# ShinYwings/SingleHDR-tf2

Hardware: AMD Instinct MI355X
Metric: HDR images/sec (512x512) end-to-end inference, deq+lin+hal (higher is better)
Workload: dtype f32

## Files before the change

### include/shdr.h

```cpp
#ifndef SHDR_H_
#define SHDR_H_

#include <stdint.h>

#ifdef __cplusplus
extern "C" {
#endif

void shdr_config_reload(void);

#define SHDR_OK          0
#define SHDR_E_SHAPE    (-1)
#define SHDR_E_ALIGN    (-2)
#define SHDR_E_ARCH     (-3)
#define SHDR_E_LAUNCH   (-4)
#define SHDR_E_NULL     (-5)

#define SHDR_ACT_NONE   0
#define SHDR_ACT_RELU   1
#define SHDR_ACT_LRELU  2
#define SHDR_ACT_TANH   3

#define SHDR_ALGO_AUTO    0
#define SHDR_ALGO_MFMA    1
// ... 163 lines not shown
                               int F, int K, void* stream);
int shdr_increase_bwd_f32(const float* rf, const float* dout, float* drf, int B, int K, void* stream);
int shdr_apply_rf_bwd_f32(const float* x, const float* rf, const float* dy, float* drf, float* dx,
                          int B, int64_t n_per_batch, int K, void* stream);
int shdr_diff_loss_f32(const float* a, const float* b, float* out, int B, int64_t n_per_sample,
                       int mode, void* stream);
int shdr_diff_loss_bwd_f32(const float* a, const float* b, const float* g, float* da, int B,
                           int64_t n_per_sample, int mode, int accumulate, void* stream);
int shdr_tv_loss_f32(const float* y, float* out, int N, int H, int W, int C, void* stream);
int shdr_tv_loss_bwd_f32(const float* y, const float* g, float* dy, int N, int H, int W, int C,
                         int accumulate, void* stream);
int shdr_logc_bwd_f32(const float* dy, const float* x, float* dx, int64_t n, void* stream);
int shdr_alpha_mask_f32(const float* x, float* alpha, int64_t npix, float thr, void* stream);
int shdr_alpha_blend_bwd_f32(const float* dA, const float* alpha, float* dhal, int64_t npix, void* stream);
int shdr_vgg_preprocess_bwd_f32(const float* dy, float* dx, int64_t npix, int in_channels, void* stream);
int shdr_adam_f32(float* p, const float* g, float* m, float* v, int64_t n, float lr_t, float beta1,
                  float beta2, float eps, float grad_scale, void* stream);

int shdr_winograd_filter_f32(const float* w, float* u, int Cin, int Cout, void* stream);
int64_t shdr_winograd_tiles(int N, int H, int W);
int shdr_winograd_input_f32(const float* x, float* v, int N, int H, int W, int C, void* stream);
int shdr_winograd_output_f32(const float* m, float* y, const float* bias, const float* scale,
                             const float* shift, int N, int H, int W, int C, int act1, int act2,
                             void* stream);

int shdr_lin_frontend_bwd_f32(const float* img, const float* dF, float* dimg, int N, int H, int W,
                              int y_channels, void* stream);
int shdr_alpha_blend_full_bwd_f32(const float* b, const float* hal, const float* dA, float* dB,
                                  float* dhal, int64_t npix, float thr, void* stream);
int shdr_unpack3_f32(const float* y, float* o0, float* o1, float* o2, float* o3, int nout,
                     int channels, int64_t npix, void* stream);
int shdr_sample_dot_f32(const float* a, const float* b, float* out, int B, int64_t n_per_sample, void* stream);
int shdr_mean_norm_fwd_f32(const float* r, const float* sum, float* out, int B, int64_t n_per_sample,
                           float eps, float target, void* stream);
int shdr_mean_norm_bwd_f32(const float* g, const float* sum, const float* gdot, float* dr, int B,
                           int64_t n_per_sample, float eps, float target, void* stream);

int shdr_act_bwd_bias_f32(const float* dy, const float* y, float* dz, float* db, float* ws, int64_t npix, int C, int act, void* stream);

int shdr_winograd_filter_packed_f32(const float* w, float* up, int Cin, int Cout, void* stream);
int shdr_conv2d_winograd_fused_f32(const float* x, const float* u, const float* bias, const float* scale,
                                   const float* shift, float* y, int N, int H, int W, int Cin, int Cout,
                                   int act1, int act2, void* stream);

int shdr_conv2d_winograd_fused2_f32(const float* x, const float* x2, const float* u, const float* bias,
                                    const float* scale, const float* shift, float* y, float* y_pool, int N, int H, int W,
                                    int C1, int C2, int Cout, int act1, int act2, void* stream);

int shdr_conv2d_winograd_fused_up2_f32(const float* x, const float* u, const float* bias, const float* scale,
                                       const float* shift, float* y, int N, int H, int W, int Cin, int Cout,
                                       int act1, int act2, void* stream);

int shdr_conv2d_x3_ok_f32(const shdr_conv2d_desc* d);
int64_t shdr_conv2d_x3_filter_elems_f32(const shdr_conv2d_desc* d);
int shdr_conv2d_x3_prepare_filter_f32(const shdr_conv2d_desc* d, const float* w, float* prepared, void* stream);
int shdr_conv2d_x3_input_absmax_f32(const float* x, int64_t n, float* prepared, void* stream);
int shdr_conv2d_fwd_x3_f32(const shdr_conv2d_desc* d, const float* x1, const float* x2, const float* prepared, const float* bias,
                           const float* scale, const float* shift, float* y, float* y_pool, void* stream);
int shdr_conv2d_fwd_x3_ranged_f32(const shdr_conv2d_desc* d, const float* x1, const float* x2, const float* prepared, const float* bias,
                                  const float* scale, const float* shift, float* y, float* y_pool, const float* x1_range,
                                  const float* x2_range, float* y_range, void* stream);
int shdr_conv2d_fwd_x3_residual_f32(const shdr_conv2d_desc* d, const float* x1, const float* x2, const float* prepared, const float* bias,
                                    const float* scale, const float* shift, const float* residual, float* y, const float* x1_range,
                                    const float* x2_range, float* y_range, void* stream);
int shdr_conv2d_fwd_x3_projected_f32(const shdr_conv2d_desc* d, const float* x1, const float* x2, const float* prepared, const float* bias,
                                     const float* scale, const float* shift, const float* proj, float* y_proj, float* y, float* y_pool,
                                     const float* x1_range, const float* x2_range, float* y_range, void* stream);
int shdr_absmax_f32(const float* x, int64_t n, float* range, void* stream);

int shdr_conv2d_x3n_ok_f32(const shdr_conv2d_desc* d);
int64_t shdr_conv2d_x3n_filter_elems_f32(const shdr_conv2d_desc* d);
int shdr_conv2d_x3n_prepare_filter_f32(const shdr_conv2d_desc* d, const float* w, float* prepared, void* stream);
int shdr_conv2d_fwd_x3n_f32(const shdr_conv2d_desc* d, const float* x1, const float* x2, const float* prepared, const float* bias,
                            const float* scale, const float* shift, const float* residual, float* y, float* y_pool, void* stream);
int shdr_conv2d_fwd_x3n_ranged_f32(const shdr_conv2d_desc* d, const float* x1, const float* x2, const float* prepared, const float* bias,
                                   const float* scale, const float* shift, const float* residual, float* y, float* y_pool,
                                   const float* x1_range, const float* x2_range, float* y_range, void* stream);

int shdr_x3_split_planes_f32(const float* x, int64_t n, const float* range, void* hi, void* lo, void* stream);
int shdr_conv2d_wgrad_x3_ok_f32(const shdr_conv2d_desc* d, int which);
int shdr_conv2d_wgrad_x3_f32(const shdr_conv2d_desc* d, const void* xh, const void* xl, int which, const void* zh, const void* zl,
                             const float* x_range, const float* z_range, float* dw, void* stream);

int shdr_conv2d_wgrad_winograd_f32(const float* x, const float* dz, float* du, float* dw, int N, int H, int W, int Cx,
                                   int Cout, int Ct, int ci_off, float x_scale, void* stream);

int shdr_u8_to_unit_f32(const uint8_t* x, float* y, int64_t npix, int reverse_channels, void* stream);
int shdr_resize_cubic_f32(const float* x, float* y, int N, int H, int W, int C, int Ho, int Wo, void* stream);
int shdr_pad_symmetric_f32(const float* x, float* y, int N, int H, int W, int C, int pad, void* stream);
int shdr_rgbe_encode_f32(const float* x, uint8_t* y, int64_t npix, int reverse_channels, void* stream);

int64_t shdr_rgbe_rle_encode(const uint8_t* rgbe, int width, int height, uint8_t* out, int64_t capacity);
int64_t shdr_rgbe_rle_decode(const uint8_t* data, int64_t size, int width, int height, uint8_t* rgbe);

#define SHDR_RLE_STAGES 4
int shdr_rgbe_rle_encode_batch_sizes(const int32_t* shapes, int n_images, int64_t* out_bytes, int64_t* workspace_bytes);
int shdr_rgbe_rle_encode_batch(const uint8_t* rgbe, const int32_t* shapes, const int32_t* shapes_dev, int n_images, uint8_t* out,
                               int64_t out_capacity, int64_t* offsets, void* workspace, void* stream);
int shdr_rgbe_rle_encode_batch_timed(const uint8_t* rgbe, const int32_t* shapes, const int32_t* shapes_dev, int n_images, uint8_t* out,
                                     int64_t out_capacity, int64_t* offsets, void* workspace, void* stream, float* stage_ms);

int shdr_hdr_load_resize_f32(const uint8_t* rgbe, float* y, int H0, int W0, int H, int W, void* stream);
int shdr_hdr_window_means_f32(const float* arena, const int64_t* offsets, const int32_t* dims, int n_files, float* partials,
                              float* means, void* stream);
int shdr_hdr_patch_sample_f32(const float* arena, const int64_t* offsets, const int32_t* dims, const float* means,
                              const int32_t* params, int param_stride, int N, int n_files, int P, float* y, void* stream);
// ... 224 lines not shown
```

### singlehdr-tf2_amd/_lib.py

```python
import ctypes
import os

_HERE = os.path.dirname(os.path.abspath(__file__))
LIB_PATH = os.environ.get("SHDR_LIB") or os.path.join(_HERE, "libshdr.so")

c_int = ctypes.c_int
c_i64 = ctypes.c_int64
c_f32 = ctypes.c_float
c_ptr = ctypes.c_void_p


class ConvDesc(ctypes.Structure):
    _fields_ = [("N", ctypes.c_int32), ("H", ctypes.c_int32), ("W", ctypes.c_int32),
                ("C1", ctypes.c_int32), ("C2", ctypes.c_int32),
                ("Cout", ctypes.c_int32), ("KH", ctypes.c_int32), ("KW", ctypes.c_int32),
                ("stride", ctypes.c_int32), ("pad_t", ctypes.c_int32), ("pad_l", ctypes.c_int32),
                ("Ho", ctypes.c_int32), ("Wo", ctypes.c_int32),
                ("x2_scale", ctypes.c_float),
                ("act1", ctypes.c_int32), ("act2", ctypes.c_int32),
                ("res_cstride", ctypes.c_int32), ("y_cstride", ctypes.c_int32),
                ("algo", ctypes.c_int32), ("cout_valid", ctypes.c_int32),
                ("w_batch_stride", ctypes.c_int64),
                ("y_pix_stride", ctypes.c_int32), ("y_off_h", ctypes.c_int32), ("y_off_w", ctypes.c_int32),
                ("y_H", ctypes.c_int32), ("y_W", ctypes.c_int32),
                ("prologue", ctypes.c_int32), ("pool", ctypes.c_int32)]


OP_CONV2D_FWD, OP_CONV2D_DGRAD, OP_CONV2D_WGRAD_WINOGRAD, OP_BATCHNORM, OP_ACT_BWD_BIAS = 0, 1, 2, 3, 4

SIGNATURES = {
    "shdr_last_error": (ctypes.c_char_p, []),
    "shdr_version": (ctypes.c_char_p, []),
    "shdr_u8_to_unit_f32": (c_int, [c_ptr, c_ptr, c_i64, c_int, c_ptr]),
    "shdr_resize_cubic_f32": (c_int, [c_ptr, c_ptr, c_int, c_int, c_int, c_int, c_int, c_int, c_ptr]),
    "shdr_pad_symmetric_f32": (c_int, [c_ptr, c_ptr, c_int, c_int, c_int, c_int, c_int, c_ptr]),
    "shdr_rgbe_encode_f32": (c_int, [c_ptr, c_ptr, c_i64, c_int, c_ptr]),
    "shdr_rgbe_rle_encode": (c_i64, [c_ptr, c_int, c_int, c_ptr, c_i64]),
    "shdr_rgbe_rle_decode": (c_i64, [c_ptr, c_i64, c_int, c_int, c_ptr]),
    "shdr_rgbe_rle_encode_batch_sizes": (c_int, [c_ptr, c_int, ctypes.POINTER(c_i64), ctypes.POINTER(c_i64)]),
    "shdr_rgbe_rle_encode_batch": (c_int, [c_ptr, c_ptr, c_ptr, c_int, c_ptr, c_i64, c_ptr, c_ptr, c_ptr]),
    "shdr_rgbe_rle_encode_batch_timed": (c_int, [c_ptr, c_ptr, c_ptr, c_int, c_ptr, c_i64, c_ptr, c_ptr, c_ptr, c_ptr]),
    "shdr_hdr_load_resize_f32": (c_int, [c_ptr, c_ptr, c_int, c_int, c_int, c_int, c_ptr]),
    "shdr_hdr_window_means_f32": (c_int, [c_ptr, c_ptr, c_ptr, c_int, c_ptr, c_ptr, c_ptr]),
    "shdr_hdr_patch_sample_f32": (c_int, [c_ptr] * 5 + [c_int] * 4 + [c_ptr, c_ptr]),
    "shdr_exr_rle_decode": (c_i64, [c_ptr, c_i64, c_ptr, c_i64]),
    "shdr_exr_unpredict_u8": (c_int, [c_ptr, c_ptr, c_i64, c_ptr, c_ptr, c_int, c_ptr]),
    "shdr_exr_load_resize_f32": (c_int, [c_ptr, c_i64, c_ptr, c_int, c_int, c_i64, c_ptr, c_ptr, c_int, c_int, c_ptr, c_int, c_int,
                                         c_int, c_ptr]),
    "shdr_deflate_huffman_host": (c_i64, [c_ptr, c_i64, c_ptr, c_i64]),
    "shdr_deflate_huffman_lengths_host": (c_int, [c_ptr, c_i64, c_ptr]),
    "shdr_deflate_huffman_batch_sizes": (c_int, [c_ptr, c_int, c_int, ctypes.POINTER(c_i64), ctypes.POINTER(c_i64)]),
    "shdr_deflate_huffman_batch": (c_int, [c_ptr, c_ptr, c_ptr, c_ptr, c_int, c_int, c_ptr, c_i64, c_ptr, c_ptr, c_ptr, c_ptr, c_ptr]),
    "shdr_deflate_lz_host": (c_i64, [c_ptr, c_i64, c_ptr, c_i64]),
    "shdr_deflate_lz_parse_host": (c_int, [c_ptr, c_i64, c_ptr]),
    "shdr_deflate_lz_batch_sizes": (c_int, [c_ptr, c_int, c_int, ctypes.POINTER(c_i64), ctypes.POINTER(c_i64)]),
    "shdr_deflate_lz_batch": (c_int, [c_ptr, c_ptr, c_ptr, c_ptr, c_int, c_int, c_ptr, c_i64, c_ptr, c_ptr, c_ptr, c_ptr, c_ptr]),
    "shdr_inflate_host": (c_i64, [c_ptr, c_i64, c_ptr, c_i64, ctypes.POINTER(c_int)]),
    "shdr_inflate_batch_sizes": (c_int, [c_ptr, c_ptr, c_int, ctypes.POINTER(c_i64), ctypes.POINTER(c_i64)]),
    "shdr_inflate_batch": (c_int, [c_ptr, c_i64, c_ptr, c_ptr, c_ptr, c_i64, c_ptr, c_ptr, c_ptr, c_int, c_ptr, c_ptr, c_ptr, c_ptr]),
    "shdr_exr_pack_sizes": (c_int, [c_ptr, c_int, c_int, c_int, ctypes.POINTER(c_i64), ctypes.POINTER(c_i64), c_ptr, c_ptr]),
    "shdr_exr_pack_f32": (c_int, [c_ptr, c_ptr, c_int, c_int, c_int, c_int, c_int, c_ptr, c_ptr, c_ptr, c_ptr, c_ptr]),
    "shdr_exr_finish_chunks": (c_int, [c_ptr, c_ptr, c_ptr, c_ptr, c_ptr, c_int, c_i64, c_int, c_ptr]),
    "shdr_philox4x32_10": (c_int, [c_ptr, c_ptr, c_ptr]),
    "shdr_camera_expose_f32": (c_int, [c_ptr, c_ptr, c_ptr, c_ptr, c_int, c_int, c_int, ctypes.c_uint64, c_ptr]),
    "shdr_jpeg_round_trip_f32": (c_int, [c_ptr] * 6 + [c_int, c_int, c_int, c_ptr]),
    "shdr_flip_rot90_f32": (c_int, [c_ptr, c_ptr, c_ptr, c_ptr, c_int, c_int, c_int, c_f32, c_ptr]),
    "shdr_pair_patch_stats": (c_int, [c_ptr, c_ptr, c_i64, c_ptr, c_ptr, c_int, c_ptr, c_ptr, c_int, c_int, c_ptr, c_ptr, c_ptr]),
    "shdr_pair_patch_gather_f32": (c_int, [c_ptr, c_ptr, c_i64, c_ptr, c_ptr, c_int, c_ptr, c_ptr, c_int, c_ptr, c_ptr, c_ptr, c_int,
                                           c_int, c_ptr, c_ptr, c_ptr]),
    "shdr_conv2d_winograd_fused_f32": (c_int, [c_ptr] * 6 + [c_int] * 7 + [c_ptr]),
    "shdr_conv2d_winograd_fused2_f32": (c_int, [c_ptr] * 8 + [c_int] * 8 + [c_ptr]),
    "shdr_conv2d_winograd_fused_up2_f32": (c_int, [c_ptr] * 6 + [c_int] * 7 + [c_ptr]),
    "shdr_conv2d_x3_ok_f32": (c_int, [ctypes.POINTER(ConvDesc)]),
    "shdr_conv2d_x3_filter_elems_f32": (c_i64, [ctypes.POINTER(ConvDesc)]),
    "shdr_conv2d_x3_prepare_filter_f32": (c_int, [ctypes.POINTER(ConvDesc), c_ptr, c_ptr, c_ptr]),
    "shdr_conv2d_fwd_x3_f32": (c_int, [ctypes.POINTER(ConvDesc)] + [c_ptr] * 9),
    "shdr_conv2d_fwd_x3_ranged_f32": (c_int, [ctypes.POINTER(ConvDesc)] + [c_ptr] * 12),
    "shdr_absmax_f32": (c_int, [c_ptr, c_i64, c_ptr, c_ptr]),
    "shdr_x3_split_planes_f32": (c_int, [c_ptr, c_i64, c_ptr, c_ptr, c_ptr, c_ptr]),
    "shdr_conv2d_wgrad_x3_ok_f32": (c_int, [ctypes.POINTER(ConvDesc), c_int]),
    "shdr_conv2d_wgrad_x3_f32": (c_int, [ctypes.POINTER(ConvDesc), c_ptr, c_ptr, c_int, c_ptr, c_ptr, c_ptr, c_ptr, c_ptr, c_ptr]),
    "shdr_config_reload": (None, []),
    "shdr_conv2d_x3_input_absmax_f32": (c_int, [c_ptr, c_i64, c_ptr, c_ptr]),
    "shdr_conv2d_x3n_ok_f32": (c_int, [ctypes.POINTER(ConvDesc)]),
    "shdr_conv2d_x3n_filter_elems_f32": (c_i64, [ctypes.POINTER(ConvDesc)]),
    "shdr_conv2d_x3n_prepare_filter_f32": (c_int, [ctypes.POINTER(ConvDesc), c_ptr, c_ptr, c_ptr]),
    "shdr_conv2d_fwd_x3n_f32": (c_int, [ctypes.POINTER(ConvDesc)] + [c_ptr] * 10),
    "shdr_conv2d_fwd_x3n_ranged_f32": (c_int, [ctypes.POINTER(ConvDesc)] + [c_ptr] * 13),
    "shdr_act_bwd_bias_f32": (c_int, [c_ptr, c_ptr, c_ptr, c_ptr, c_ptr, c_i64, c_int, c_int, c_ptr]),
    "shdr_winograd_filter_packed_f32": (c_int, [c_ptr, c_ptr, c_int, c_int, c_ptr]),
    "shdr_conv2d_wgrad_winograd_f32": (c_int, [c_ptr] * 4 + [c_int] * 7 + [c_f32, c_ptr]),
    "shdr_crc32c": (ctypes.c_uint32, [c_ptr, ctypes.c_uint64, ctypes.c_uint32]),
    "shdr_same_pad": (c_int, [c_int, c_int, c_int, ctypes.POINTER(c_int), ctypes.POINTER(c_int)]),
    "shdr_conv2d_fwd_f32": (c_int, [ctypes.POINTER(ConvDesc)] + [c_ptr] * 9),
    "shdr_conv2d_fwd_yrange_f32": (c_int, [ctypes.POINTER(ConvDesc)] + [c_ptr] * 10),
    "shdr_conv2d_plan_f32": (c_int, [ctypes.POINTER(ConvDesc), c_int]),
    "shdr_conv2d_prepared_filter_elems_f32": (c_i64, [ctypes.POINTER(ConvDesc), c_int]),
    "shdr_conv2d_filter_is_plain_f32": (c_int, [ctypes.POINTER(ConvDesc), c_int]),
    "shdr_conv2d_prepare_filter_f32": (c_int, [ctypes.POINTER(ConvDesc), c_int, c_ptr, c_ptr, c_ptr]),
    "shdr_conv2d_workspace_bytes_f32": (c_i64, [ctypes.POINTER(ConvDesc), c_int]),
    "shdr_conv2d_fwd_prepared_f32": (c_int, [ctypes.POINTER(ConvDesc)] + [c_ptr] * 11),
    "shdr_conv2d_fwd_prepared_ranged_f32": (c_int, [ctypes.POINTER(ConvDesc)] + [c_ptr] * 14),
    "shdr_conv2d_projected_ok_f32": (c_int, [ctypes.POINTER(ConvDesc)]),
    "shdr_conv2d_fwd_prepared_projected_f32": (c_int, [ctypes.POINTER(ConvDesc)] + [c_ptr] * 15),
    "shdr_conv2d_up2_lowres_ok_f32": (c_int, [ctypes.POINTER(ConvDesc)]),
    "shdr_conv2d_up2_lowres_filter_elems_f32": (c_i64, [ctypes.POINTER(ConvDesc)]),
    "shdr_conv2d_up2_lowres_prepare_filter_f32": (c_int, [ctypes.POINTER(ConvDesc), c_ptr, c_ptr, c_ptr]),
    "shdr_conv2d_up2_lowres_workspace_bytes_f32": (c_i64, [ctypes.POINTER(ConvDesc)]),
    "shdr_conv2d_fwd_up2_lowres_f32": (c_int, [ctypes.POINTER(ConvDesc)] + [c_ptr] * 10),
    "shdr_conv2d_up2_fused_ok_f32": (c_int, [ctypes.POINTER(ConvDesc)]),
    "shdr_conv2d_up2_narrow_enabled": (c_int, []),
    "shdr_conv2d_up2_fused_filter_elems_f32": (c_i64, [ctypes.POINTER(ConvDesc)]),
    "shdr_conv2d_up2_fused_prepare_filter_f32": (c_int, [ctypes.POINTER(ConvDesc), c_ptr, c_ptr, c_ptr]),
    "shdr_conv2d_fwd_up2_fused_f32": (c_int, [ctypes.POINTER(ConvDesc)] + [c_ptr] * 11),
    "shdr_conv2d_fwd_x3_projected_f32": (c_int, [ctypes.POINTER(ConvDesc)] + [c_ptr] * 14),
    "shdr_conv2d_fwd_x3_residual_f32": (c_int, [ctypes.POINTER(ConvDesc)] + [c_ptr] * 12),
    "shdr_conv2d_dgrad_workspace_bytes_f32": (c_i64, [ctypes.POINTER(ConvDesc), c_int]),
    "shdr_conv2d_dgrad_f32": (c_int, [ctypes.POINTER(ConvDesc), c_int, c_ptr, c_ptr, c_ptr, c_ptr, c_ptr]),
    "shdr_conv2d_dgrad_tracks_range_f32": (c_int, [ctypes.POINTER(ConvDesc), c_int]),
    "shdr_conv2d_dgrad_ranged_f32": (c_int, [ctypes.POINTER(ConvDesc), c_int, c_ptr, c_ptr, c_ptr, c_ptr, c_ptr, c_ptr, c_ptr]),
    "shdr_workspace_bytes": (c_i64, [c_int, ctypes.POINTER(ConvDesc), c_int]),
    "shdr_soft_hist_bwd_f32": (c_int, [c_ptr, c_ptr, c_ptr, c_i64, c_int, c_int, c_ptr]),
    "shdr_conv2d_wgrad_f32": (c_int, [ctypes.POINTER(ConvDesc), c_ptr, c_int, c_ptr, c_ptr, c_ptr]),
    "shdr_filter_transform_f32": (c_int, [c_ptr, c_ptr, c_int, c_int, c_int, c_int, c_int, c_int, c_f32, c_ptr]),
    "shdr_bias_grad_f32": (c_int, [c_ptr, c_ptr, c_i64, c_int, c_ptr]),
    "shdr_soft_hist_fwd_f32": (c_int, [c_ptr, c_ptr, c_i64, c_int, c_int, c_ptr]),
# ... 128 lines not shown
```

### singlehdr-tf2_amd/csrc/conv_x3.hip

```cpp
#include <hip/hip_fp16.h>
#include <stdlib.h>

#include <type_traits>

#include "shdr_internal.h"

namespace {

using f32x4 = __attribute__((ext_vector_type(4))) float;
using f16x8 = __attribute__((ext_vector_type(8))) _Float16;
using f16x4 = __attribute__((ext_vector_type(4))) _Float16;
using u32x4 = __attribute__((ext_vector_type(4))) unsigned;

constexpr int X3_HEADER_FLOATS = 16;
constexpr int BN = 64, NT = 4, MT = 4;
constexpr int IMG_HALVES = BN * 32;
constexpr int UNIT_HALVES = 2 * IMG_HALVES;
constexpr int LRW = 10, LRPIX = LRW * LRW;
constexpr int LRJ = (LRPIX * 8 + 255) / 256;
template <int KH, int KW>
struct X3G {
  static constexpr int PH = 16 + KH - 1, PWID = 16 + KW - 1, PPIX = PH * PWID;
  static constexpr int PJ = (PPIX * 8 + 255) / 256;
  static constexpr int PATCH_HALVES = PPIX * 32;
// ... 458 lines not shown
  }
    if (LOOK == 1) {
      {
        const int kh = 0;
#pragma unroll
        for (int kw = 0; kw < KW; ++kw) X3_TAP(true)
      }
#pragma unroll 1
      for (int kh = 1; kh < (MP ? kh_n : KH); ++kh) {
#pragma unroll
        for (int kw = 0; kw < KW; ++kw) X3_TAP(false)
      }
    } else {
#pragma unroll
      for (int kh = 0; kh < KH; ++kh) {
#pragma unroll
        for (int kw = 0; kw < KW; ++kw) X3_TAP(kh == 0)
      }
      asm volatile("s_waitcnt vmcnt(0)" : "+v"(fr[0][0]), "+v"(fr[0][1]) : : "memory");
#pragma unroll
      for (int j = 0; j < FJ; ++j) fr[NFR - 1][j] = fr[0][j];
    }
#undef X3_TAP
#undef X3_SLOT
    if (c + 1 < nch) {
      if (UP) {
        park_lr();
        __syncthreads();
      } else {
        __syncthreads();
      }
      store_patch(nxt);
    }
  };
#pragma unroll 1
  for (int c = 0; c < nch; c += DEPTH) {
    chunk(c, Set0{}, Set1{});
    if (DEPTH == 2 && c + 1 < nch) chunk(c + 1, Set1{}, Set0{});
  }
  }
#undef pr
#undef X3_WAIT_VM

  x3_tile_epilogue<4, true>(a, acc, img, oh0 + wave * MT, ow0 + pc, pc, fg, n0, ixs, lane, wave,
                            reinterpret_cast<unsigned*>(reinterpret_cast<char*>(xsm) + (UP ? G::LDS_BYTES_UP : G::LDS_BYTES)));
}

#undef patch_h
#undef patch_l
#undef filt
#undef lrs

constexpr int X1_BP = 128;
template <int NS>
__global__ __launch_bounds__(256, 2) void conv_x3_1x1_kernel(const X3Args a) {
  constexpr int MT1 = 2 * NS, BP = X1_BP;
  constexpr int PJ1 = BP * 8 / 256;
  constexpr int IMG = BP * 32;
  static_assert(NS * (BP / (MT1 * 16)) == 4, "four waves: NS cout slices x pixel groups");
  __shared__ __attribute__((aligned(16))) _Float16 x1sm[2 * 2 * IMG];
  __shared__ unsigned x1rw[4];

  const int tid = threadIdx.x, lane = tid & 63;
  const int wave = __builtin_amdgcn_readfirstlane(tid >> 6);
  const int slice = wave % NS, grp = wave / NS;
  const int L = xcd_remap(blockIdx.x, a.nblk_m * a.nblk_n);
  const int pn = L % a.nblk_n, pm = L / a.nblk_n;
  const int P0 = pm * BP, Ptot = a.N * a.H * a.W;

  int ppix[PJ1];
  const int pdst = (tid >> 3) * 32 + 8 * (((tid & 7) >> 1) ^ sx((tid >> 3) & 15)) + 4 * (tid & 1);
#pragma unroll
  for (int j = 0; j < PJ1; ++j) {
    const int P = P0 + (tid >> 3) + 32 * j;
    ppix[j] = -1;
    if (P < Ptot) {
      const int ow = P % a.W, t = P / a.W;
      const int oh = t % a.H, img = t / a.H;
      const int ih = a.in_s * oh + a.bh, iw = a.in_s * ow + a.bw;
      if ((unsigned)ih < (unsigned)a.Hin && (unsigned)iw < (unsigned)a.Win) ppix[j] = (img * a.Hin + ih) * a.Win + iw;
    }
  }
  const int nch1 = a.C1 >> 5, nch = (a.C1 + a.C2) >> 5;
  using Set0 = std::integral_constant<int, 0>;
  using Set1 = std::integral_constant<int, 1>;
  f32x4 pr_sets[2][PJ1];
  auto load_patch = [&](int c, auto setc) __attribute__((always_inline)) {
    constexpr int S = decltype(setc)::value;
    const bool second = c >= nch1;
    const float* src = second ? a.x2 : a.x1;
    const int Cs = second ? a.C2 : a.C1;
    const int c0 = (second ? c - nch1 : c) << 5;
#pragma unroll
    for (int j = 0; j < PJ1; ++j) {
      pr_sets[S][j] = (f32x4){0.f, 0.f, 0.f, 0.f};
      if (ppix[j] >= 0) pr_sets[S][j] = *reinterpret_cast<const f32x4*>(src + (size_t)(unsigned)ppix[j] * (unsigned)Cs + c0 + 4 * (tid & 7));
    }
  };
  float xs = 1.0f, ixs = 1.0f;
  auto store_patch = [&](int buf, auto setc) __attribute__((always_inline)) {
    constexpr int S = decltype(setc)::value;
#pragma unroll
    for (int j = 0; j < PJ1; ++j) {
      unsigned h[2], l[2];
      x3_split4(pr_sets[S][j], xs, h, l);
      *reinterpret_cast<uint2*>(x1sm + buf * 2 * IMG + pdst + 1024 * j) = make_uint2(h[0], h[1]);
      *reinterpret_cast<uint2*>(x1sm + buf * 2 * IMG + IMG + pdst + 1024 * j) = make_uint2(l[0], l[1]);
    }
  };
  const int fi = lane & 15, fg = lane >> 4;
  const _Float16* wsl = a.wp + (size_t)(pn * NS + slice) * nch * UNIT_HALVES + fi * 32 + 8 * fg;
  f16x8 f0h[2], f0l[2], f1h[2], f1l[2];
  auto load_w = [&](int c, int half, f16x8 (&h)[2], f16x8 (&l)[2]) __attribute__((always_inline)) {
    const _Float16* g = wsl + (size_t)c * UNIT_HALVES + half * 2 * 16 * 32;
#pragma unroll
    for (int k = 0; k < 2; ++k) {
      h[k] = *reinterpret_cast<const f16x8*>(g + k * 16 * 32);
      l[k] = *reinterpret_cast<const f16x8*>(g + IMG_HALVES + k * 16 * 32);
    }
  };

  f32x4 acc[MT1][NT];
#pragma unroll
  for (int mi = 0; mi < MT1; ++mi)
#pragma unroll
    for (int ni = 0; ni < NT; ++ni) acc[mi][ni] = (f32x4){0.f, 0.f, 0.f, 0.f};
  const int pc = pcol(fi);
  const int a_rd = (grp * MT1 * 16 + pc) * 32 + 8 * (fg ^ sx(pc));

  auto half_pass = [&](int buf, auto halfc, const f16x8 (&wh)[2], const f16x8 (&wl)[2]) __attribute__((always_inline)) {
    constexpr int H = decltype(halfc)::value;
    const int bo = buf * 2 * IMG + a_rd;
    f16x8 ws[2], ph[2], pl[2];
    auto read_a = [&](int mi, int slot) __attribute__((always_inline)) {
      ph[slot] = *reinterpret_cast<const f16x8*>(x1sm + bo + mi * 16 * 32);
      pl[slot] = *reinterpret_cast<const f16x8*>(x1sm + IMG + bo + mi * 16 * 32);
    };
    read_a(0, 0);
#pragma unroll
    for (int k = 0; k < 2; ++k) ws[k] = wh[k] * (_Float16)(1.0f / 2048.0f);
#pragma unroll
    for (int mi = 0; mi < MT1; ++mi) {
      if (mi + 1 < MT1) read_a(mi + 1, (mi + 1) & 1);
      __builtin_amdgcn_sched_barrier(0);
#pragma unroll
      for (int k = 0; k < 2; ++k) acc[mi][2 * H + k] = __builtin_amdgcn_mfma_f32_16x16x32_f16(wh[k], ph[mi & 1], acc[mi][2 * H + k], 0, 0, 0);
#pragma unroll
      for (int k = 0; k < 2; ++k) acc[mi][2 * H + k] = __builtin_amdgcn_mfma_f32_16x16x32_f16(ws[k], pl[mi & 1], acc[mi][2 * H + k], 0, 0, 0);
#pragma unroll
      for (int k = 0; k < 2; ++k) acc[mi][2 * H + k] = __builtin_amdgcn_mfma_f32_16x16x32_f16(wl[k], ph[mi & 1], acc[mi][2 * H + k], 0, 0, 0);
      __builtin_amdgcn_sched_barrier(0);
    }
  };
  using Half0 = std::integral_constant<int, 0>;
  using Half1 = std::integral_constant<int, 1>;

  load_patch(0, Set0{});
  if (nch > 1) load_patch(1, Set1{});
  load_w(0, 0, f0h, f0l);
  x3_range_scale(a.xr1, a.xr2, xs, ixs);
  store_patch(0, Set0{});
  if (nch > 2) load_patch(2, Set0{});
  auto chunk = [&](int c, auto nxt) __attribute__((always_inline)) {
    __syncthreads();
    load_w(c, 1, f1h, f1l);
    if (c + 1 < nch) {
      store_patch((c + 1) & 1, nxt);
      if (c + 3 < nch) load_patch(c + 3, nxt);
    }
    half_pass(c & 1, Half0{}, f0h, f0l);
    if (c + 1 < nch) load_w(c + 1, 0, f0h, f0l);
    half_pass(c & 1, Half1{}, f1h, f1l);
  };
#pragma unroll 1
  for (int c = 0; c < nch; c += 2) {
    chunk(c, Set1{});
    if (c + 1 < nch) chunk(c + 1, Set0{});
  }

  const float inv_s = a.hdr[1] * ixs;
  const unsigned yr_seen = a.yr ? __hip_atomic_load(a.yr, __ATOMIC_RELAXED, __HIP_MEMORY_SCOPE_AGENT) : 0u;
  int ep0 = (pn * NS + slice) * BN;
  asm volatile("" : "+s"(ep0));
  f32x4 bias_r[NT], scale_r[NT], shift_r[NT];
#pragma unroll
  for (int ni = 0; ni < NT; ++ni) {
    const int cl = ni * 16 + 4 * fg;
    bias_r[ni] = a.bias ? *reinterpret_cast<const f32x4*>(a.bias + ep0 + cl) : (f32x4){0.f, 0.f, 0.f, 0.f};
    scale_r[ni] = a.scale ? *reinterpret_cast<const f32x4*>(a.scale + ep0 + cl) : (f32x4){1.f, 1.f, 1.f, 1.f};
    shift_r[ni] = a.scale ? *reinterpret_cast<const f32x4*>(a.shift + ep0 + cl) : (f32x4){0.f, 0.f, 0.f, 0.f};
  }
  const int Pw = P0 + grp * MT1 * 16 + pc;
  float ym = 0.0f;
  constexpr int EB = 4;
#pragma unroll
  for (int m0 = 0; m0 < MT1; m0 += EB) {
    f32x4 res_r[EB][NT];
    if (a.res) {
#pragma unroll
      for (int e = 0; e < EB; ++e)
#pragma unroll
        for (int ni = 0; ni < NT; ++ni) {
          const int P = Pw + 16 * (m0 + e);
          res_r[e][ni] = P < Ptot ? *reinterpret_cast<const f32x4*>(a.res + (size_t)P * a.res_cs + ep0 + ni * 16 + 4 * fg) : (f32x4){0.f, 0.f, 0.f, 0.f};
        }
    }
#pragma unroll
    for (int e = 0; e < EB; ++e) {
      const int P = Pw + 16 * (m0 + e);
      if (P0 + grp * MT1 * 16 + 16 * (m0 + e) >= Ptot) continue;
#pragma unroll
      for (int ni = 0; ni < NT; ++ni) {
        f32x4 v = acc[m0 + e][ni] * inv_s;
        asm("" : "+v"(v));
        v += bias_r[ni];
        shdr::act_apply4<0>(v, a.act1);
        if (a.scale) v = v * scale_r[ni] + shift_r[ni];
        if (a.res) v += res_r[e][ni];
        shdr::act_apply4<0>(v, a.act2);
        if (P < Ptot) {
          *reinterpret_cast<f32x4*>(a.y + (size_t)P * a.Cout + ep0 + ni * 16 + 4 * fg) = v;
          if (a.yr) ym = fmaxf(fmaxf(fmaxf(fmaxf(ym, fabsf(v[0])), fabsf(v[1])), fabsf(v[2])), fabsf(v[3]));
        }
      }
    }
  }
  if (a.yr) x3_range_out(a.yr, ym, lane, wave, yr_seen, x1rw);
}

constexpr int XW_THREADS = 512, XW_BN = 128;
constexpr long XW_UP_MIN_COUT = 128;
struct XWG {
  using G = X3G<3, 3>;
  static constexpr int PJ = (G::PPIX * 8 + XW_THREADS - 1) / XW_THREADS;
  static constexpr int RANGE_BYTES = 32;
  static constexpr int LR_BYTES = LRPIX * 32 * 4;
  static constexpr int LDS_BYTES = (2 * 2 * G::PATCH_HALVES + 2 * 2 * UNIT_HALVES) * 2;
};
template <bool UP>
__global__ __launch_bounds__(XW_THREADS, 2) void conv_x3_wide_kernel(const X3Args a) {
  using G = X3G<3, 3>;
  constexpr int KH = 3, KW = 3, PWID = G::PWID, PPIX = G::PPIX, PJ = XWG::PJ, PATCH_HALVES = G::PATCH_HALVES, NTAPS = 9;
  static_assert((PJ - 1) * XW_THREADS < PPIX * 8 && PJ == 6, "every piece but the last is inside the patch for every thread");
  extern __shared__ __attribute__((aligned(16))) _Float16 xsm[];
#define patch_buf(B) (xsm + (B) * 2 * PATCH_HALVES)
#define filt (xsm + 4 * PATCH_HALVES)
#define lrs (reinterpret_cast<float*>(xsm + 4 * PATCH_HALVES + 4 * UNIT_HALVES))

  const int tid = threadIdx.x, lane = tid & 63;
  const int wave = __builtin_amdgcn_readfirstlane(tid >> 6);
  const int slice = wave >> 2, wq = wave & 3;
  const int L = xcd_remap(blockIdx.x, a.nblk_m * a.nblk_n);
  const int pn = L % a.nblk_n;
  int pm = L / a.nblk_n;
  const int tx = pm % a.tiles_x;
  pm /= a.tiles_x;
  const int ty = pm % a.tiles_y;
  const int img = pm / a.tiles_y;
  const int n0 = pn * XW_BN + slice * BN, oh0 = ty * 16, ow0 = tx * 16;

  constexpr int PL = UP ? (LRPIX * 8 + XW_THREADS - 1) / XW_THREADS : PJ;
  constexpr int T0 = UP ? 4 : 3;
  int ppix[PL], pdst[PJ];
  int pcnt = 0;
  if (UP) {
#pragma unroll
    for (int j = 0; j < PL; ++j) {
      const int p = tid + XW_THREADS * j;
      const int pix = p >> 3;
      const int ly = pix / LRW, lx = pix - ly * LRW;
      const int r = (oh0 >> 1) - 1 + ly, c = (ow0 >> 1) - 1 + lx;
      ppix[j] = (pix < LRPIX && (unsigned)r < (unsigned)a.Hl && (unsigned)c < (unsigned)a.Wl) ? (img * a.Hl + r) * a.Wl + c : -1;
      pcnt += __ballot(ppix[j] >= 0) != 0ull;
    }
  }
#pragma unroll
  for (int j = 0; j < (UP ? 0 : PJ); ++j) {
    const int p = tid + XW_THREADS * j;
    const int pix = p >> 3, q = p & 7;
    const int py = pix / PWID, px = pix - py * PWID;
// ... 282 lines not shown
    const int ta = t2 / TW, tb = t2 - TW * ta;
    const int tap = (p0 + step * ta) * KWF + (q0 + step * tb);
    const int ch = chunk * 32 + k;
    float v = nb * 64 + co < Cout ? w[((size_t)tap * Ct + ch) * Cout + nb * 64 + co] * s : 0.0f;
    if (ch >= C1) v *= x2_scale;
    const _Float16 h = (_Float16)v;
    _Float16* o = out + ((size_t)(nb * nunits + u) * 2) * IMG_HALVES + co * 32 + k;
    o[0] = h;
    o[IMG_HALVES] = (_Float16)(v - (float)h);
  }
}

}

namespace {

struct X3Phase { int th, tw, p0, q0, step, bh, bw; };
int x3_phases(const shdr_conv2d_desc* d, X3Phase ph[4]) {
  if (d->stride == 1 || d->KH == 1) {
    ph[0] = X3Phase{d->KH, d->KW, 0, 0, d->stride, -d->pad_t, -d->pad_l};
    return 1;
  }
  int n = 0;
  for (int p0 = 0; p0 < 2; ++p0)
    for (int q0 = 0; q0 < 2; ++q0) ph[n++] = X3Phase{(d->KH - p0 + 1) / 2, (d->KW - q0 + 1) / 2, p0, q0, 2, p0 - d->pad_t, q0 - d->pad_l};
  return n;
}
inline int64_t x3_phase_floats(const X3Phase& p, int Ct, int Cout) { return X3_HEADER_FLOATS + (int64_t)p.th * p.tw * Ct * ((Cout + 63) / 64 * 64); }

template <bool UP, int KH, int KW, bool MP, int LOOK>
int launch_x3_look(const X3Args& a, hipStream_t st) {
  constexpr int lds = (UP ? X3G<KH, KW>::LDS_BYTES_UP : X3G<KH, KW>::LDS_BYTES) + X3G<KH, KW>::RANGE_BYTES;
  static bool attr_done[shdr::kMaxDevices] = {};
  const int dev_slot = shdr::device_slot();
  if (!attr_done[dev_slot]) {
    hipError_t e = hipFuncSetAttribute(reinterpret_cast<const void*>(&conv_x3_kernel<UP, KH, KW, MP, LOOK>), hipFuncAttributeMaxDynamicSharedMemorySize, lds);
    if (e != hipSuccess) return shdr::fail(SHDR_E_ARCH, "hipFuncSetAttribute: %s", hipGetErrorString(e));
    attr_done[dev_slot] = true;
  }
  const long nblk = (long)a.nblk_m * a.nblk_n;
  if (nblk > 0x7fffffffL) return shdr::fail(SHDR_E_SHAPE, "conv2d_x3: grid of %ld blocks", nblk);
  hipLaunchKernelGGL((conv_x3_kernel<UP, KH, KW, MP, LOOK>), dim3((unsigned)nblk), dim3(256), lds, st, a);
  return shdr::check_launch("conv_x3_kernel");
}
template <bool UP, int KH, int KW, bool MP = false>
int launch_x3(const X3Args& a, hipStream_t st) {
  int look = 2;
  if (const char* e = SHDR_ENV("SHDR_X3_LOOK")) look = atoi(e);
  constexpr bool look2 = KH == 3 && KW == 3 && !MP;
  if (look >= 2 && look2) return launch_x3_look<UP, KH, KW, MP, look2 ? 2 : 1>(a, st);
  return launch_x3_look<UP, KH, KW, MP, 1>(a, st);
}

int launch_x3_1x1(const X3Args& a0, hipStream_t st) {
  X3Args a = a0;
  const long npix = (long)a.N * a.H * a.W;
  const int ns = a.Cout % 256 == 0 ? 4 : 2;
  a.nblk_m = (int)((npix + X1_BP - 1) / X1_BP);
  a.nblk_n = a.Cout / (64 * ns);
  const long nblk = (long)a.nblk_m * a.nblk_n;
  if (nblk > 0x7fffffffL) return shdr::fail(SHDR_E_SHAPE, "conv2d_x3: grid of %ld blocks", nblk);
  if (ns == 4) hipLaunchKernelGGL((conv_x3_1x1_kernel<4>), dim3((unsigned)nblk), dim3(256), 0, st, a);
  else hipLaunchKernelGGL((conv_x3_1x1_kernel<2>), dim3((unsigned)nblk), dim3(256), 0, st, a);
  return shdr::check_launch("conv_x3_1x1_kernel");
}

template <bool UP>
int launch_x3_wide(const X3Args& a0, hipStream_t st) {
  X3Args a = a0;
  a.nblk_n = a.Cout / XW_BN;
  constexpr int lds = XWG::LDS_BYTES + (UP ? XWG::LR_BYTES : 0) + XWG::RANGE_BYTES;
  static bool attr_done[shdr::kMaxDevices] = {};
  const int dev_slot = shdr::device_slot();
  if (!attr_done[dev_slot]) {
    hipError_t e = hipFuncSetAttribute(reinterpret_cast<const void*>(&conv_x3_wide_kernel<UP>), hipFuncAttributeMaxDynamicSharedMemorySize, lds);
    if (e != hipSuccess) return shdr::fail(SHDR_E_ARCH, "hipFuncSetAttribute: %s", hipGetErrorString(e));
    attr_done[dev_slot] = true;
  }
  const long nblk = (long)a.nblk_m * a.nblk_n;
  if (nblk > 0x7fffffffL) return shdr::fail(SHDR_E_SHAPE, "conv2d_x3: grid of %ld blocks", nblk);
  hipLaunchKernelGGL((conv_x3_wide_kernel<UP>), dim3((unsigned)nblk), dim3(XW_THREADS), lds, st, a);
  return shdr::check_launch("conv_x3_wide_kernel");
}

}

extern "C" int shdr_conv2d_x3_ok_f32(const shdr_conv2d_desc* d) {
  if (!d || d->C1 <= 0 || d->C1 % 32 || d->C2 % 32 || (d->Cout % 64 && (d->Cout != 32 || d->stride != 1 || SHDR_ENV("SHDR_NO_X3_COUT32")))) return 0;
  const int cv = d->cout_valid > 0 ? d->cout_valid : d->Cout;
  if (cv != d->Cout || d->w_batch_stride != 0 || d->y_pix_stride > 1) return 0;
  if ((long)d->N * d->H * d->W * (d->C1 > d->C2 ? d->C1 : d->C2) >= (1L << 31)) return 0;
  if (SHDR_ENV("SHDR_NO_X3")) return 0;
  if (d->act1 == SHDR_ACT_TANH || d->act2 == SHDR_ACT_TANH) return 0;
  if (d->stride == 1) {
    const bool k3 = d->KH == 3 && d->KW == 3 && d->pad_t == 1 && d->pad_l == 1;
    int k1_min = 64;
    if (const char* e = SHDR_ENV("SHDR_X3_1X1_MIN_K")) k1_min = atoi(e);
    const bool k1 = d->KH == 1 && d->KW == 1 && d->pad_t == 0 && d->pad_l == 0 && d->C1 + d->C2 >= k1_min && SHDR_ENV("SHDR_NO_X3_1X1") == nullptr;
    if (!(k3 || k1) || d->Ho != d->H || d->Wo != d->W) return 0;
  } else if (d->stride == 2 && d->KH == 1 && d->KW == 1) {
    if (d->pad_t != 0 || d->pad_l != 0 || d->C2 != 0 || d->prologue != SHDR_PROLOGUE_NONE || d->Ho != (d->H + 1) / 2 || d->Wo != (d->W + 1) / 2 ||
        d->C1 < 64 || SHDR_ENV("SHDR_NO_X3_1X1") || SHDR_ENV("SHDR_NO_X3_STRIDE2"))
      return 0;
  } else {
    int ho = 0, wo = 0, pt = 0, pl = 0;
    shdr_same_pad(d->H, 7, 2, &ho, &pt);
    shdr_same_pad(d->W, 7, 2, &wo, &pl);
    if (d->stride != 2 || d->KH != 7 || d->KW != 7 || d->C2 != 0 || d->prologue != SHDR_PROLOGUE_NONE || d->Ho != ho || d->Wo != wo || d->pad_t != pt ||
        d->pad_l != pl || SHDR_ENV("SHDR_NO_X3_STRIDE2"))
      return 0;
  }
  const long blocks = (long)d->N * ((d->Ho + 15) / 16) * ((d->Wo + 15) / 16) * ((d->Cout + 63) / 64);
  long min_blocks = 192;
  if (const char* e = SHDR_ENV("SHDR_X3_MIN_BLOCKS")) min_blocks = atol(e);
  return blocks >= min_blocks ? 1 : 0;
}

extern "C" int64_t shdr_conv2d_x3_filter_elems_f32(const shdr_conv2d_desc* d) {
  if (!d || d->C1 <= 0 || (d->C1 + d->C2) % 32 || (d->Cout % 64 && d->Cout != 32) || (d->stride != 1 && d->stride != 2)) return -1;
  X3Phase ph[4];
  const int n = x3_phases(d, ph);
  int64_t total = 0;
  for (int i = 0; i < n; ++i) total += x3_phase_floats(ph[i], d->C1 + d->C2, d->Cout);
  return total;
}

extern "C" int shdr_conv2d_x3_prepare_filter_premax_f32(const shdr_conv2d_desc* d, const float* w, float* prepared, int premax, void* stream);
extern "C" int shdr_conv2d_x3_prepare_filter_f32(const shdr_conv2d_desc* d, const float* w, float* prepared, void* stream) {
  return shdr_conv2d_x3_prepare_filter_premax_f32(d, w, prepared, 0, stream);
}
extern "C" int shdr_conv2d_x3_prepare_filter_premax_f32(const shdr_conv2d_desc* d, const float* w, float* prepared, int premax, void* stream) {
  SHDR_REQUIRE(d && w && prepared, SHDR_E_NULL, "conv2d_x3_prepare_filter: null pointer");
  const int Ct = d->C1 + d->C2;
  SHDR_REQUIRE(Ct > 0 && Ct % 32 == 0 && d->C1 % 32 == 0 && d->Cout > 0 && (d->Cout % 64 == 0 || d->Cout == 32), SHDR_E_SHAPE,
               "conv2d_x3_prepare_filter: need C %% 32 == 0, Cout %% 64 == 0 (or Cout 32)");
  SHDR_REQUIRE(shdr::aligned16(prepared), SHDR_E_ALIGN, "conv2d_x3_prepare_filter: prepared must be 16-byte aligned");
  hipStream_t st = reinterpret_cast<hipStream_t>(stream);
// ... 139 lines not shown
```

Measured before the change: 944.6.

## Make 1x1 x3 conv kernel persistent with next-tile prefetch under epilogue

Turns the 1x1 MFMA conv kernel into a persistent kernel. It launches about two blocks per CU for small-K/small-N shapes and loops over tiles with a grid stride. When there is no residual (and, for NS=4, no scale), it loads the next tile's patch and weights while the current tile's epilogue runs. The aim is to hide global-load latency and cut block launch and tail overhead. In exchange it raises register pressure, adds per-tile re-setup, and adds grid-size heuristics with environment overrides.

Measured after the change: 949.8, median of 5. Within noise of the previous version (+0.5%).

```diff
diff --git a/include/shdr.h b/include/shdr.h
--- a/include/shdr.h
+++ b/include/shdr.h
@@ -239,6 +239,7 @@
                                        int act1, int act2, void* stream);
 
 int shdr_conv2d_x3_ok_f32(const shdr_conv2d_desc* d);
+int shdr_conv2d_x3_1x1_grid(int64_t npix, int cin, int cout);
 int64_t shdr_conv2d_x3_filter_elems_f32(const shdr_conv2d_desc* d);
 int shdr_conv2d_x3_prepare_filter_f32(const shdr_conv2d_desc* d, const float* w, float* prepared, void* stream);
 int shdr_conv2d_x3_input_absmax_f32(const float* x, int64_t n, float* prepared, void* stream);
diff --git a/singlehdr-tf2_amd/_lib.py b/singlehdr-tf2_amd/_lib.py
--- a/singlehdr-tf2_amd/_lib.py
+++ b/singlehdr-tf2_amd/_lib.py
@@ -72,6 +72,7 @@
     "shdr_conv2d_winograd_fused2_f32": (c_int, [c_ptr] * 8 + [c_int] * 8 + [c_ptr]),
     "shdr_conv2d_winograd_fused_up2_f32": (c_int, [c_ptr] * 6 + [c_int] * 7 + [c_ptr]),
     "shdr_conv2d_x3_ok_f32": (c_int, [ctypes.POINTER(ConvDesc)]),
+    "shdr_conv2d_x3_1x1_grid": (c_int, [c_i64, c_int, c_int]),
     "shdr_conv2d_x3_filter_elems_f32": (c_i64, [ctypes.POINTER(ConvDesc)]),
     "shdr_conv2d_x3_prepare_filter_f32": (c_int, [ctypes.POINTER(ConvDesc), c_ptr, c_ptr, c_ptr]),
     "shdr_conv2d_fwd_x3_f32": (c_int, [ctypes.POINTER(ConvDesc)] + [c_ptr] * 9),
diff --git a/singlehdr-tf2_amd/csrc/conv_x3.hip b/singlehdr-tf2_amd/csrc/conv_x3.hip
--- a/singlehdr-tf2_amd/csrc/conv_x3.hip
+++ b/singlehdr-tf2_amd/csrc/conv_x3.hip
@@ -534,40 +534,60 @@
 #undef lrs
 
 constexpr int X1_BP = 128;
-template <int NS>
-__global__ __launch_bounds__(256, 2) void conv_x3_1x1_kernel(const X3Args a) {
+template <int NS, bool LOOK>
+__device__ __forceinline__ void x3_1x1_tiles(const X3Args& a, _Float16* x1sm, unsigned* x1rw) {
   constexpr int MT1 = 2 * NS, BP = X1_BP;
   constexpr int PJ1 = BP * 8 / 256;
   constexpr int IMG = BP * 32;
   static_assert(NS * (BP / (MT1 * 16)) == 4, "four waves: NS cout slices x pixel groups");
-  __shared__ __attribute__((aligned(16))) _Float16 x1sm[2 * 2 * IMG];
-  __shared__ unsigned x1rw[4];
-
-  const int tid = threadIdx.x, lane = tid & 63;
-  const int wave = __builtin_amdgcn_readfirstlane(tid >> 6);
+
+  const int wave = __builtin_amdgcn_readfirstlane(threadIdx.x >> 6);
   const int slice = wave % NS, grp = wave / NS;
-  const int L = xcd_remap(blockIdx.x, a.nblk_m * a.nblk_n);
-  const int pn = L % a.nblk_n, pm = L / a.nblk_n;
-  const int P0 = pm * BP, Ptot = a.N * a.H * a.W;
-
-  int ppix[PJ1];
-  const int pdst = (tid >> 3) * 32 + 8 * (((tid & 7) >> 1) ^ sx((tid >> 3) & 15)) + 4 * (tid & 1);
-#pragma unroll
-  for (int j = 0; j < PJ1; ++j) {
-    const int P = P0 + (tid >> 3) + 32 * j;
-    ppix[j] = -1;
-    if (P < Ptot) {
-      const int ow = P % a.W, t = P / a.W;
-      const int oh = t % a.H, img = t / a.H;
-      const int ih = a.in_s * oh + a.bh, iw = a.in_s * ow + a.bw;
-      if ((unsigned)ih < (unsigned)a.Hin && (unsigned)iw < (unsigned)a.Win) ppix[j] = (img * a.Hin + ih) * a.Win + iw;
-    }
-  }
+  auto thread_id = [&]() __attribute__((always_inline)) {
+    int l;
+    asm volatile("v_mbcnt_lo_u32_b32 %0, -1, 0\n\tv_mbcnt_hi_u32_b32 %0, -1, %0" : "=v"(l));
+    return wave * 64 + l;
+  };
+  const int ntiles = a.nblk_m * a.nblk_n, Ptot = a.N * a.H * a.W;
   const int nch1 = a.C1 >> 5, nch = (a.C1 + a.C2) >> 5;
+
+  int pn = 0, P0 = 0;
+  int ppix[PJ1], pq4 = 0;
+  const _Float16* wsl = nullptr;
+  auto set_tile = [&](int tl) __attribute__((always_inline)) {
+    const int tv = thread_id();
+    int W = a.W, H = a.H, nbn = a.nblk_n;
+    asm volatile("" : "+s"(tl), "+s"(W), "+s"(H), "+s"(nbn));
+    pq4 = 4 * (tv & 7);
+    const int L = xcd_remap(tl, ntiles);
+    pn = L % nbn;
+    P0 = (L / nbn) * BP;
+#pragma unroll
+    for (int j = 0; j < PJ1; ++j) {
+      const int P = P0 + (tv >> 3) + 32 * j;
+      ppix[j] = -1;
+      if (P < Ptot) {
+        const int ow = P % W, t = P / W;
+        const int oh = t % H, img = t / H;
+        const int ih = a.in_s * oh + a.bh, iw = a.in_s * ow + a.bw;
+        if ((unsigned)ih < (unsigned)a.Hin && (unsigned)iw < (unsigned)a.Win) ppix[j] = (img * a.Hin + ih) * a.Win + iw;
+      }
+    }
+    wsl = a.wp + (size_t)(pn * NS + slice) * nch * UNIT_HALVES + (tv & 15) * 32 + 8 * ((tv & 63) >> 4);
+  };
+  int fi = 0, fg = 0, pc = 0, pdst = 0, a_rd = 0;
+  auto set_lane = [&]() __attribute__((always_inline)) {
+    const int tv = thread_id();
+    fi = tv & 15;
+    fg = (tv & 63) >> 4;
+    pc = pcol(fi);
+    pdst = (tv >> 3) * 32 + 8 * (((tv & 7) >> 1) ^ sx((tv >> 3) & 15)) + 4 * (tv & 1);
+    a_rd = (grp * MT1 * 16 + pc) * 32 + 8 * (fg ^ sx(pc));
+  };
   using Set0 = std::integral_constant<int, 0>;
   using Set1 = std::integral_constant<int, 1>;
   f32x4 pr_sets[2][PJ1];
-  auto load_patch = [&](int c, auto setc) __attribute__((always_inline)) {
+  auto load_patch = [&](int c, auto setc, bool on = true) __attribute__((always_inline)) {
     constexpr int S = decltype(setc)::value;
     const bool second = c >= nch1;
     const float* src = second ? a.x2 : a.x1;
@@ -576,7 +596,7 @@
 #pragma unroll
     for (int j = 0; j < PJ1; ++j) {
       pr_sets[S][j] = (f32x4){0.f, 0.f, 0.f, 0.f};
-      if (ppix[j] >= 0) pr_sets[S][j] = *reinterpret_cast<const f32x4*>(src + (size_t)(unsigned)ppix[j] * (unsigned)Cs + c0 + 4 * (tid & 7));
+      if (on && ppix[j] >= 0) pr_sets[S][j] = *reinterpret_cast<const f32x4*>(src + (size_t)(unsigned)ppix[j] * (unsigned)Cs + c0 + pq4);
     }
   };
   float xs = 1.0f, ixs = 1.0f;
@@ -590,8 +610,6 @@
       *reinterpret_cast<uint2*>(x1sm + buf * 2 * IMG + IMG + pdst + 1024 * j) = make_uint2(l[0], l[1]);
     }
   };
-  const int fi = lane & 15, fg = lane >> 4;
-  const _Float16* wsl = a.wp + (size_t)(pn * NS + slice) * nch * UNIT_HALVES + fi * 32 + 8 * fg;
   f16x8 f0h[2], f0l[2], f1h[2], f1l[2];
   auto load_w = [&](int c, int half, f16x8 (&h)[2], f16x8 (&l)[2]) __attribute__((always_inline)) {
     const _Float16* g = wsl + (size_t)c * UNIT_HALVES + half * 2 * 16 * 32;
@@ -603,12 +621,6 @@
   };
 
   f32x4 acc[MT1][NT];
-#pragma unroll
-  for (int mi = 0; mi < MT1; ++mi)
-#pragma unroll
-    for (int ni = 0; ni < NT; ++ni) acc[mi][ni] = (f32x4){0.f, 0.f, 0.f, 0.f};
-  const int pc = pcol(fi);
-  const int a_rd = (grp * MT1 * 16 + pc) * 32 + 8 * (fg ^ sx(pc));
 
   auto half_pass = [&](int buf, auto halfc, const f16x8 (&wh)[2], const f16x8 (&wl)[2]) __attribute__((always_inline)) {
     constexpr int H = decltype(halfc)::value;
@@ -637,12 +649,11 @@
   using Half0 = std::integral_constant<int, 0>;
   using Half1 = std::integral_constant<int, 1>;
 
-  load_patch(0, Set0{});
-  if (nch > 1) load_patch(1, Set1{});
-  load_w(0, 0, f0h, f0l);
-  x3_range_scale(a.xr1, a.xr2, xs, ixs);
-  store_patch(0, Set0{});
-  if (nch > 2) load_patch(2, Set0{});
+  auto head = [&]() __attribute__((always_inline)) {
+    load_patch(0, Set0{});
+    load_patch(1, Set1{}, nch > 1);
+    load_w(0, 0, f0h, f0l);
+  };
   auto chunk = [&](int c, auto nxt) __attribute__((always_inline)) {
     __syncthreads();
     load_w(c, 1, f1h, f1l);
@@ -654,60 +665,117 @@
     if (c + 1 < nch) load_w(c + 1, 0, f0h, f0l);
     half_pass(c & 1, Half1{}, f1h, f1l);
   };
-#pragma unroll 1
-  for (int c = 0; c < nch; c += 2) {
-    chunk(c, Set1{});
-    if (c + 1 < nch) chunk(c + 1, Set0{});
-  }
-
-  const float inv_s = a.hdr[1] * ixs;
-  const unsigned yr_seen = a.yr ? __hip_atomic_load(a.yr, __ATOMIC_RELAXED, __HIP_MEMORY_SCOPE_AGENT) : 0u;
-  int ep0 = (pn * NS + slice) * BN;
-  asm volatile("" : "+s"(ep0));
-  f32x4 bias_r[NT], scale_r[NT], shift_r[NT];
-#pragma unroll
-  for (int ni = 0; ni < NT; ++ni) {
-    const int cl = ni * 16 + 4 * fg;
-    bias_r[ni] = a.bias ? *reinterpret_cast<const f32x4*>(a.bias + ep0 + cl) : (f32x4){0.f, 0.f, 0.f, 0.f};
-    scale_r[ni] = a.scale ? *reinterpret_cast<const f32x4*>(a.scale + ep0 + cl) : (f32x4){1.f, 1.f, 1.f, 1.f};
-    shift_r[ni] = a.scale ? *reinterpret_cast<const f32x4*>(a.shift + ep0 + cl) : (f32x4){0.f, 0.f, 0.f, 0.f};
-  }
-  const int Pw = P0 + grp * MT1 * 16 + pc;
+
   float ym = 0.0f;
-  constexpr int EB = 4;
-#pragma unroll
-  for (int m0 = 0; m0 < MT1; m0 += EB) {
-    f32x4 res_r[EB][NT];
-    if (a.res) {
-#pragma unroll
-      for (int e = 0; e < EB; ++e)
+  auto epilogue = [&](int epn, int eP0, auto scalec, auto resc, auto&& under) __attribute__((always_inline)) {
+    const bool has_scale = decltype(scalec)::value && a.scale, has_res = decltype(resc)::value && a.res;
+    const float inv_s = a.hdr[1] * ixs;
+    int ep0 = (epn * NS + slice) * BN;
+    asm volatile("" : "+s"(ep0));
+    f32x4 bias_r[NT], scale_r[NT], shift_r[NT];
+#pragma unroll
+    for (int ni = 0; ni < NT; ++ni) {
+      const int cl = ni * 16 + 4 * fg;
+      bias_r[ni] = a.bias ? *reinterpret_cast<const f32x4*>(a.bias + ep0 + cl) : (f32x4){0.f, 0.f, 0.f, 0.f};
+      scale_r[ni] = has_scale ? *reinterpret_cast<const f32x4*>(a.scale + ep0 + cl) : (f32x4){1.f, 1.f, 1.f, 1.f};
+      shift_r[ni] = has_scale ? *reinterpret_cast<const f32x4*>(a.shift + ep0 + cl) : (f32x4){0.f, 0.f, 0.f, 0.f};
+    }
+    if (LOOK) {
+#pragma unroll
+      for (int ni = 0; ni < NT; ++ni) asm volatile("" : "+v"(bias_r[ni]), "+v"(scale_r[ni]), "+v"(shift_r[ni]));
+    }
+    under();
+    const int Pw = eP0 + grp * MT1 * 16 + pc;
+    constexpr int EB = NS == 4 ? 2 : 4;
+#pragma unroll
+    for (int m0 = 0; m0 < MT1; m0 += EB) {
+      f32x4 res_r[EB][NT];
+      if (has_res) {
+#pragma unroll
+        for (int e = 0; e < EB; ++e)
+#pragma unroll
+          for (int ni = 0; ni < NT; ++ni) {
+            const int P = Pw + 16 * (m0 + e);
+            res_r[e][ni] = P < Ptot ? *reinterpret_cast<const f32x4*>(a.res + (size_t)P * a.res_cs + ep0 + ni * 16 + 4 * fg) : (f32x4){0.f, 0.f, 0.f, 0.f};
+          }
+      }
+#pragma unroll
+      for (int e = 0; e < EB; ++e) {
+        const int P = Pw + 16 * (m0 + e);
+        if (eP0 + grp * MT1 * 16 + 16 * (m0 + e) >= Ptot) continue;
 #pragma unroll
         for (int ni = 0; ni < NT; ++ni) {
-          const int P = Pw + 16 * (m0 + e);
-          res_r[e][ni] = P < Ptot ? *reinterpret_cast<const f32x4*>(a.res + (size_t)P * a.res_cs + ep0 + ni * 16 + 4 * fg) : (f32x4){0.f, 0.f, 0.f, 0.f};
-        }
-    }
-#pragma unroll
-    for (int e = 0; e < EB; ++e) {
-      const int P = Pw + 16 * (m0 + e);
-      if (P0 + grp * MT1 * 16 + 16 * (m0 + e) >= Ptot) continue;
-#pragma unroll
-      for (int ni = 0; ni < NT; ++ni) {
-        f32x4 v = acc[m0 + e][ni] * inv_s;
-        asm("" : "+v"(v));
-        v += bias_r[ni];
-        shdr::act_apply4<0>(v, a.act1);
-        if (a.scale) v = v * scale_r[ni] + shift_r[ni];
-        if (a.res) v += res_r[e][ni];
-        shdr::act_apply4<0>(v, a.act2);
-        if (P < Ptot) {
-          *reinterpret_cast<f32x4*>(a.y + (size_t)P * a.Cout + ep0 + ni * 16 + 4 * fg) = v;
-          if (a.yr) ym = fmaxf(fmaxf(fmaxf(fmaxf(ym, fabsf(v[0])), fabsf(v[1])), fabsf(v[2])), fabsf(v[3]));
+          f32x4 v = acc[m0 + e][ni] * inv_s;
+          asm("" : "+v"(v));
+          v += bias_r[ni];
+          shdr::act_apply4<0>(v, a.act1);
+          if (has_scale) v = v * scale_r[ni] + shift_r[ni];
+          if (has_res) v += res_r[e][ni];
+          shdr::act_apply4<0>(v, a.act2);
+          if (P < Ptot) {
+            *reinterpret_cast<f32x4*>(a.y + (size_t)P * a.Cout + ep0 + ni * 16 + 4 * fg) = v;
+            if (a.yr) ym = fmaxf(fmaxf(fmaxf(fmaxf(ym, fabsf(v[0])), fabsf(v[1])), fabsf(v[2])), fabsf(v[3]));
+          }
         }
       }
     }
-  }
-  if (a.yr) x3_range_out(a.yr, ym, lane, wave, yr_seen, x1rw);
+  };
+  using Yes = std::integral_constant<bool, true>;
+  using No = std::integral_constant<bool, false>;
+
+  unsigned yr_seen = 0u;
+  int tl = blockIdx.x;
+  set_tile(tl);
+  head();
+  x3_range_scale(a.xr1, a.xr2, xs, ixs);
+#pragma unroll 1
+  for (;;) {
+    const int epn = pn, eP0 = P0;
+    set_lane();
+    store_patch(0, Set0{});
+    if (nch > 2) load_patch(2, Set0{});
+#pragma unroll
+    for (int mi = 0; mi < MT1; ++mi)
+#pragma unroll
+      for (int ni = 0; ni < NT; ++ni) acc[mi][ni] = (f32x4){0.f, 0.f, 0.f, 0.f};
+#pragma unroll 1
+    for (int c = 0; c < nch; c += 2) {
+      chunk(c, Set1{});
+      if (c + 1 < nch) chunk(c + 1, Set0{});
+    }
+    tl += gridDim.x;
+    const bool more = tl < ntiles;
+    if (more) asm volatile("s_waitcnt lgkmcnt(0)\n\ts_barrier" ::: "memory");
+    else if (a.yr) yr_seen = __hip_atomic_load(a.yr, __ATOMIC_RELAXED, __HIP_MEMORY_SCOPE_AGENT);
+    auto next_head = [&]() __attribute__((always_inline)) {
+      if (LOOK && more) {
+        set_tile(tl);
+        head();
+      }
+    };
+    if (!LOOK) {
+#pragma unroll
+      for (int j = 0; j < PJ1; ++j) pr_sets[0][j] = pr_sets[1][j] = (f32x4){0.f, 0.f, 0.f, 0.f};
+#pragma unroll
+      for (int k = 0; k < 2; ++k) f0h[k] = f0l[k] = f1h[k] = f1l[k] = (f16x8){0, 0, 0, 0, 0, 0, 0, 0};
+    }
+    if (!LOOK) epilogue(epn, eP0, Yes{}, Yes{}, next_head);
+    else if (NS == 2) epilogue(epn, eP0, Yes{}, No{}, next_head);
+    else epilogue(epn, eP0, No{}, No{}, next_head);
+    if (!more) break;
+    if (!LOOK) {
+      set_tile(tl);
+      head();
+    }
+  }
+  if (a.yr) x3_range_out(a.yr, ym, thread_id() & 63, wave, yr_seen, x1rw);
+}
+template <int NS>
+__global__ __launch_bounds__(256, 2) void conv_x3_1x1_kernel(const X3Args a) {
+  __shared__ __attribute__((aligned(16))) _Float16 x1sm[2 * 2 * X1_BP * 32];
+  __shared__ unsigned x1rw[4];
+  if (!a.res && (NS == 2 || !a.scale)) x3_1x1_tiles<NS, true>(a, x1sm, x1rw);
+  else x3_1x1_tiles<NS, false>(a, x1sm, x1rw);
 }
 
 constexpr int XW_THREADS = 512, XW_BN = 128;
@@ -1096,16 +1164,34 @@
   return launch_x3_look<UP, KH, KW, MP, 1>(a, st);
 }
 
+int x3_1x1_grid(long ntiles, int K, int BN) {
+  if (const char* e = SHDR_ENV("SHDR_X3_1X1_ONESHOT"))
+    if (atoi(e) != 0) return (int)ntiles;
+  long cap = 0;
+  if (const char* e = SHDR_ENV("SHDR_X3_1X1_GRID")) cap = atol(e);
+  if (cap <= 0 && (long)K * BN >= 100L * (K + BN)) return (int)ntiles;
+  static int cus[shdr::kMaxDevices] = {};
+  const int dev_slot = shdr::device_slot();
+  if (cus[dev_slot] <= 0) {
+    int dev = 0, n = 0;
+    if (hipGetDevice(&dev) != hipSuccess || hipDeviceGetAttribute(&n, hipDeviceAttributeMultiprocessorCount, dev) != hipSuccess || n < 1) return (int)ntiles;
+    cus[dev_slot] = n;
+  }
+  long g = 2L * cus[dev_slot];
+  if (cap > 0 && cap < g) g = cap;
+  return (int)(ntiles < g ? ntiles : g);
+}
 int launch_x3_1x1(const X3Args& a0, hipStream_t st) {
   X3Args a = a0;
   const long npix = (long)a.N * a.H * a.W;
   const int ns = a.Cout % 256 == 0 ? 4 : 2;
   a.nblk_m = (int)((npix + X1_BP - 1) / X1_BP);
   a.nblk_n = a.Cout / (64 * ns);
-  const long nblk = (long)a.nblk_m * a.nblk_n;
-  if (nblk > 0x7fffffffL) return shdr::fail(SHDR_E_SHAPE, "conv2d_x3: grid of %ld blocks", nblk);
-  if (ns == 4) hipLaunchKernelGGL((conv_x3_1x1_kernel<4>), dim3((unsigned)nblk), dim3(256), 0, st, a);
-  else hipLaunchKernelGGL((conv_x3_1x1_kernel<2>), dim3((unsigned)nblk), dim3(256), 0, st, a);
+  const long ntiles = (long)a.nblk_m * a.nblk_n;
+  if (ntiles > 0x7fffffffL) return shdr::fail(SHDR_E_SHAPE, "conv2d_x3: grid of %ld blocks", ntiles);
+  const dim3 grid((unsigned)x3_1x1_grid(ntiles, a.C1 + a.C2, 64 * ns));
+  if (ns == 4) hipLaunchKernelGGL((conv_x3_1x1_kernel<4>), grid, dim3(256), 0, st, a);
+  else hipLaunchKernelGGL((conv_x3_1x1_kernel<2>), grid, dim3(256), 0, st, a);
   return shdr::check_launch("conv_x3_1x1_kernel");
 }
 
@@ -1127,6 +1213,12 @@
   return shdr::check_launch("conv_x3_wide_kernel");
 }
 
+}
+
+extern "C" int shdr_conv2d_x3_1x1_grid(int64_t npix, int cin, int cout) {
+  if (npix <= 0 || cin <= 0 || cin % 32 || cout <= 0 || cout % 128) return 0;
+  const int ns = cout % 256 == 0 ? 4 : 2;
+  return x3_1x1_grid((npix + X1_BP - 1) / X1_BP * (cout / (64 * ns)), cin, 64 * ns);
 }
 
 extern "C" int shdr_conv2d_x3_ok_f32(const shdr_conv2d_desc* d) {
```
